# HiLab-git/FPL-plus

Hardware: AMD Instinct MI355X
Metric: 3D volumes/sec (train step, 80x160x160) (higher is better)
Workload: dtype bf16; 1 GPU; UNet3D-DSBN 32-base-ch bf16 (fp32 master weights), per-GPU batch 2x1x80x160x160 synthetic VS crops, DiceLoss + Adam, domain alternating per step; global_batch=2, parallelism=dp1, step=zero_grad+forward+loss+backward+allreduce+adam

## Files before the change

### fpl-plus_amd/csrc/common.h

```cpp
#pragma once
#include <hip/hip_runtime.h>
#include <math.h>
#include <stdint.h>
#include <stdio.h>
#include <stdarg.h>
#include <string.h>
#include "../../include/fplx.h"

typedef __bf16 bf16_t;

#define FPLX_WAVE 64

inline char* fplx_err_buf() {
  static thread_local char buf[512];
  return buf;
}
inline int fplx_fail(int code, const char* fmt, ...) {
  va_list ap;
  va_start(ap, fmt);
  vsnprintf(fplx_err_buf(), 512, fmt, ap);
  va_end(ap);
  return code;
}
inline int fplx_check_launch(const char* what) {
// ... 194 lines not shown
  FPLX_REQUIRE((need < 1 || s0) && (need < 2 || s1), FPLX_E_NULL, "%s: kind %d needs %d state buffer(s) here", who, kind, need);
  *ns = need;
  return FPLX_OK;
}
struct FplxBlock { int x, y, z; };
__device__ __forceinline__ FplxBlock fplx_xcd_block(int on) {
  FplxBlock b = {(int)blockIdx.x, (int)blockIdx.y, (int)blockIdx.z};
  if (!on) return b;
  const unsigned gx = gridDim.x, gy = gridDim.y, gz = gridDim.z, t = gx * gy * gz;
  const unsigned l = (blockIdx.z * gy + blockIdx.y) * gx + blockIdx.x;
  const unsigned xcd = l & 7u, q = t >> 3, r = t & 7u;
  const unsigned lp = xcd * q + (xcd < r ? xcd : r) + (l >> 3);
  const unsigned per = gy * gz, xq = lp / per, rem = lp - xq * per;
  b.x = __builtin_amdgcn_readfirstlane((int)xq);
  b.z = __builtin_amdgcn_readfirstlane((int)(rem / gy));
  b.y = __builtin_amdgcn_readfirstlane((int)(rem % gy));
  return b;
}
struct FplxTileRange { int64_t first, end, step; };
__device__ __forceinline__ FplxTileRange fplx_xcd_tiles(int64_t ntiles, int on) {
  FplxTileRange t = {(int64_t)blockIdx.x, ntiles, (int64_t)gridDim.x};
  if (!on || gridDim.x < 16) return t;
  const unsigned c = blockIdx.x & 7u, xcd = (blockIdx.y * gridDim.x + blockIdx.x) & 7u;
  const int64_t q = ntiles >> 3, r = ntiles & 7;
  const int64_t start = xcd * q + ((int64_t)xcd < r ? xcd : r);
  t.first = start + (blockIdx.x >> 3);
  t.end = start + q + ((int64_t)xcd < r ? 1 : 0);
  t.step = (gridDim.x - c + 7u) >> 3;
  return t;
}
template <typename... P, typename... A>
inline void fplx_launch(void (*kernel)(P...), dim3 grid, dim3 block, size_t lds, hipStream_t st, A... args) {
  if (lds) (void)hipFuncSetAttribute((const void*)kernel, hipFuncAttributeMaxDynamicSharedMemorySize, (int)lds);
  kernel<<<grid, block, lds, st>>>(args...);
}
#endif
#define FPLX_KNOB_LIST(X)                                                                                              \
  X(XCD, "xcd", 1)                                                    \
  X(BRICK, "brick", 1)                                    \
  X(BRICK_FILL, "brick_fill", 192)           \
  X(BRICK_GEO, "brick_geo", -1)                    \
  X(BRICK_KSPLIT, "brick_ksplit", 0)                                             \
  X(EDGE_BLOCKS, "edge_blocks", 1024)                             \
  X(STEM_ROWS, "stem_rows", 1)                                              \
  X(OUTCONV_T, "outconv_t", 1)                                 \
  X(OUTCONV_DGRAD_MFMA, "outconv_dgrad_mfma", 1)                                                                       \
  X(OUTCONV_FWD_ROWS, "outconv_fwd_rows", 1)  \
  X(OUTCONV_DGRAD_ROWS, "outconv_dgrad_rows", 1)  \
  X(PACK_TILED, "pack_tiled", 1)                                                                                       \
  X(PACK_MULTI, "pack_multi", 1)                                                                                       \
  X(MARCH, "march", 1)                           \
  X(MARCH64_FW, "march64_fw", 0)                                \
  X(MARCH_DS, "march_ds", 0)                                       \
  X(MARCH128, "march128", 1)                                                                                           \
  X(MARCH64_LW, "march64_lw", 1)            \
  X(MARCH32_V2, "march32_v2", 4)              \
  X(WG_COT_MINVOX, "wg_cot_minvox", 0)                                                                                 \
  X(WG_TW, "wg_tw", 0)                                                                                                 \
  X(WG_CIT, "wg_cit", 2)                                                                                               \
  X(WG_COT, "wg_cot", 2)                                                                                               \
  X(WG_DS, "wg_ds", 0)                                                                                                 \
  X(WG_VOX, "wg_vox", 1)                              \
  X(WG_ROLL, "wg_roll", 1)                     \
  X(WG_ROLL_GEO, "wg_roll_geo", 0)          \
  X(WG_ROLL_M16, "wg_roll_m16", 1)                 \
  X(WG_ROLL_MB, "wg_roll_mb", 1)            \
  X(WG_ROLL_CUS, "wg_roll_cus", 256)                                \
  X(WG_ROLL_OVH, "wg_roll_ovh", 9)                     \
  X(WG_ROLL_MINVOX, "wg_roll_minvox", 0)                                                   \
  X(WG_ROLL2D, "wg_roll2d", 1)              \
  X(WG_ROLL2D_OVH, "wg_roll2d_ovh", 3)      \
  X(WG_REDUCE_ROWS, "wg_reduce_rows", 8)    \
  X(WG_VOX_LW, "wg_vox_lw", 1)              \
  X(WG_VOX_CUS, "wg_vox_cus", 128)          \
  X(WG_VOX_MAXV, "wg_vox_maxv", 10000)         \
  X(TILE_NT, "tile_nt", 0)                                                                                             \
  X(TILE_KS, "tile_ks", 0)                                                                                             \
  X(MID_TILE, "mid_tile", 1)                                                                                           \
  X(DECONV_ROWS, "deconv_rows", 1)                                                                                     \
  X(DECONV_DGRAD_ROWS, "deconv_dgrad_rows", 1)   \
  X(ROWS_SMALL_DIV, "rows_small_div", 16)   \
  X(EW_GROUP, "ew_group", 1)                                                                                           \
  X(POOL_COL, "pool_col", 1)                         \
  X(EW_INFLIGHT, "ew_inflight", 2)          \
  X(EW_INFLIGHT_REDUCE, "ew_inflight_reduce", 2)
enum FplxKnobId {
#define FPLX_KNOB_ENUM(id, key, def) FPLX_K_##id,
  FPLX_KNOB_LIST(FPLX_KNOB_ENUM)
#undef FPLX_KNOB_ENUM
  FPLX_K_COUNT
};
extern "C" __attribute__((visibility("hidden"))) int64_t fplx_knob_values[FPLX_K_COUNT];
static inline int64_t fplx_knob(int id) { return __atomic_load_n(&fplx_knob_values[id], __ATOMIC_RELAXED); }
static inline int fplx_xcd_on() { return (int)fplx_knob(FPLX_K_XCD); }

static inline int fplx_rows_for(int64_t voxels) {
  constexpr int cap = 512;
  const int div = voxels <= 32768 ? (int)fplx_knob(FPLX_K_ROWS_SMALL_DIV) : 64;
  int64_t r = (voxels + div - 1) / div;
  if (r > cap) r = cap;
  if (r < 1) r = 1;
  return (int)r;
}
```

### fpl-plus_amd/csrc/elementwise.hip

```cpp
#include "common.h"
#include "philox.h"

namespace {

constexpr int EW_THREADS = 256;

template <typename T> struct Vec;
template <> struct Vec<float> {
  static constexpr int N = 4;
  typedef float4 raw;
  static __device__ __forceinline__ void load(const float* p, float (&v)[4]) {
    const float4 r = *reinterpret_cast<const float4*>(p);
    v[0] = r.x; v[1] = r.y; v[2] = r.z; v[3] = r.w;
  }
  static __device__ __forceinline__ void load_nt(const float* p, float (&v)[4]) { load(p, v); }
  static __device__ __forceinline__ void store(float* p, const float (&v)[4]) {
    *reinterpret_cast<float4*>(p) = make_float4(v[0], v[1], v[2], v[3]);
  }
};
template <> struct Vec<bf16_t> {
  static constexpr int N = 8;
  typedef __attribute__((ext_vector_type(8))) __bf16 raw;
  static __device__ __forceinline__ void load(const bf16_t* p, float (&v)[8]) {
    const raw r = *reinterpret_cast<const raw*>(p);
#pragma unroll
    for (int i = 0; i < 8; ++i) v[i] = (float)r[i];
  }
  static __device__ __forceinline__ void load_nt(const bf16_t* p, float (&v)[8]) {
    const raw r = __builtin_nontemporal_load(reinterpret_cast<const raw*>(p));
#pragma unroll
    for (int i = 0; i < 8; ++i) v[i] = (float)r[i];
  }
  static __device__ __forceinline__ void store(bf16_t* p, const float (&v)[8]) {
    raw r;
#pragma unroll
    for (int i = 0; i < 8; ++i) r[i] = (bf16_t)v[i];
    *reinterpret_cast<raw*>(p) = r;
  }
};

template <typename T, int VEC>
__device__ __forceinline__ void ldv(const T* p, float (&v)[VEC]) {
  if constexpr (VEC == 1) v[0] = Act<T>::ld(p);
  else Vec<T>::load(p, v);
}
template <typename T, int VEC>
__device__ __forceinline__ void ldv_nt(const T* p, float (&v)[VEC]) {
  if constexpr (VEC == 1) v[0] = Act<T>::ld(p);
  else Vec<T>::load_nt(p, v);
}
template <typename T, int VEC>
__device__ __forceinline__ void stv(T* p, const float (&v)[VEC]) {
  if constexpr (VEC == 1) Act<T>::st(p, v[0]);
  else Vec<T>::store(p, v);
}

template <int VEC>
__device__ __forceinline__ void keep_flags(int64_t e, uint32_t thr, uint32_t k0, uint32_t k1, uint32_t sid,
                                           bool (&keep)[VEC]) {
  if constexpr (VEC == 1) {
    const Philox4 r = philox4x32_10((uint32_t)(e >> 2), 0u, sid, 0u, k0, k1);
    keep[0] = r.v[e & 3] >= thr;
  } else {
#pragma unroll
    for (int g = 0; g < VEC / 4; ++g) {
      const Philox4 r = philox4x32_10((uint32_t)((e >> 2) + g), 0u, sid, 0u, k0, k1);
#pragma unroll
      for (int i = 0; i < 4; ++i) keep[g * 4 + i] = r.v[i] >= thr;
    }
  }
}

struct DropCfg { uint32_t thr, k0, k1, sid; float inv_keep; int on; };

inline DropCfg make_drop(float p, uint64_t seed, uint32_t sid) {
  DropCfg d;
  d.on = p > 0.f;
  d.thr = dropout_threshold(p);
  d.k0 = (uint32_t)seed;
  d.k1 = (uint32_t)(seed >> 32);
  d.sid = sid;
  d.inv_keep = d.on ? (float)(1.0 / (1.0 - (double)p)) : 1.f;
  return d;
}

constexpr int FIN_THREADS = 256;
__global__ void __launch_bounds__(FIN_THREADS)
bn_train_finalize_k(const float* __restrict__ stats, int rows, int C, double count,
                    const float* __restrict__ gamma, const float* __restrict__ beta,
                    float* __restrict__ rm, float* __restrict__ rv, int64_t* __restrict__ nbt,
                    float momentum, float eps, float* __restrict__ mean, float* __restrict__ rstd,
                    float* __restrict__ scale, float* __restrict__ shift) {
  const int c = blockIdx.x;
  double s1 = 0.0, s2 = 0.0;
  for (int r = threadIdx.x; r < rows; r += FIN_THREADS) {
    s1 += (double)stats[((int64_t)r * 2 + 0) * C + c];
    s2 += (double)stats[((int64_t)r * 2 + 1) * C + c];
  }
  s1 = wave_sum_d(s1);
  s2 = wave_sum_d(s2);
  __shared__ double wred[FIN_THREADS / 64][2];
  if ((threadIdx.x & 63) == 0) { wred[threadIdx.x >> 6][0] = s1; wred[threadIdx.x >> 6][1] = s2; }
  __syncthreads();
  if (threadIdx.x != 0) return;
  s1 = (wred[0][0] + wred[1][0]) + (wred[2][0] + wred[3][0]);
  s2 = (wred[0][1] + wred[1][1]) + (wred[2][1] + wred[3][1]);
  if (c == 0 && nbt) *nbt += 1;
  const double m = s1 / count;
  double var = s2 / count - m * m;
  if (var < 0.0) var = 0.0;
  const float rs = (float)(1.0 / sqrt(var + (double)eps));
  const float mf = (float)m;
  mean[c] = mf;
  rstd[c] = rs;
  const float sc = gamma[c] * rs;
  scale[c] = sc;
  shift[c] = beta[c] - mf * sc;
  if (rm) rm[c] = (1.f - momentum) * rm[c] + momentum * mf;
  if (rv) {
    const double unb = count > 1.0 ? var * count / (count - 1.0) : var;
    rv[c] = (1.f - momentum) * rv[c] + momentum * (float)unb;
  }
}

__global__ void bn_eval_prepare_k(const float* __restrict__ gamma, const float* __restrict__ beta,
                                  const float* __restrict__ rm, const float* __restrict__ rv, float eps, int C,
                                  float* __restrict__ scale, float* __restrict__ shift) {
  const int c = blockIdx.x * blockDim.x + threadIdx.x;
  if (c >= C) return;
  const float rs = 1.0f / sqrtf(rv[c] + eps);
  const float sc = gamma[c] * rs;
  scale[c] = sc;
  shift[c] = beta[c] - rm[c] * sc;
}

template <typename T, int VEC>
__global__ void __launch_bounds__(EW_THREADS)
bn_act_fwd_k(const T* __restrict__ y, int64_t ldy, T* __restrict__ out, int64_t ldo, const float* __restrict__ scale,
// ... 538 lines not shown
  __shared__ float red[EW_THREADS / 64 * 64][2 * VEC + 1];
  float* row = part + (int64_t)blockIdx.x * (2 * C + 1);
  for (int ofs = G; ofs < 64; ofs <<= 1) {
#pragma unroll
    for (int j = 0; j < VEC; ++j) { sdz[j] += __shfl_xor(sdz[j], ofs, 64); sdx[j] += __shfl_xor(sdx[j], ofs, 64); }
    sds += __shfl_xor(sds, ofs, 64);
  }
  const int lane = threadIdx.x & 63, wave = threadIdx.x >> 6;
  if (lane < G) {
#pragma unroll
    for (int j = 0; j < VEC; ++j) { red[wave * 64 + lane][j] = sdz[j]; red[wave * 64 + lane][VEC + j] = sdx[j]; }
    red[wave * 64 + lane][2 * VEC] = sds;
  }
  __syncthreads();
  if ((int)threadIdx.x < G) {
#pragma unroll
    for (int j = 0; j < VEC; ++j) {
      float t0 = 0.f, t1 = 0.f;
#pragma unroll
      for (int wv = 0; wv < EW_THREADS / 64; ++wv) { t0 += red[wv * 64 + threadIdx.x][j]; t1 += red[wv * 64 + threadIdx.x][VEC + j]; }
      row[c0 + j] = t0;
      row[C + c0 + j] = t1;
    }
  }
  if (threadIdx.x == 0) {
    float t = 0.f;
    for (int wv = 0; wv < EW_THREADS / 64; ++wv)
      for (int k = 0; k < G; ++k) t += red[wv * 64 + k][2 * VEC];
    row[2 * C] = t;
  }
}

template <typename T, int VEC>
__global__ void __launch_bounds__(EW_THREADS)
bn_act_pool_fwd_col_k(const T* __restrict__ y, int64_t ldy, T* __restrict__ out, int64_t ldo, T* __restrict__ pooled,
                      int64_t ldp, const float* __restrict__ scale, const float* __restrict__ shift,
                      const float* __restrict__ slope_p, int N, int D, int H, int W, int C, int pd) {
  const int G = C / VEC, VL = EW_THREADS / G;
  const int g = threadIdx.x % G, vl = threadIdx.x / G, c0 = g * VEC;
  const int Do = D / pd, Ho = H / 2;
  const unsigned units = (unsigned)N * Do * Ho * W;
  const float slope = *slope_p;
  float sc[VEC], sh[VEC];
#pragma unroll
  for (int j = 0; j < VEC; ++j) { sc[j] = scale[c0 + j]; sh[j] = shift[c0 + j]; }
  for (unsigned u = blockIdx.x * VL + vl; u < units; u += gridDim.x * VL) {
    unsigned q = u;
    const int w = (int)(q % (unsigned)W); q /= (unsigned)W;
    const int ho = (int)(q % (unsigned)Ho); q /= (unsigned)Ho;
    const int d_o = (int)(q % (unsigned)Do);
    const int64_t n = q / (unsigned)Do;
    float a[4][VEC], best[VEC];
    int64_t vis[4];
#pragma unroll
    for (int t = 0; t < 4; ++t) {
      if (t >= 2 * pd) break;
      vis[t] = ((n * D + pd * d_o + (t >> 1)) * H + 2 * ho + (t & 1)) * W + w;
      ldv_nt<T, VEC>(y + vis[t] * ldy + c0, a[t]);
    }
#pragma unroll
    for (int j = 0; j < VEC; ++j) best[j] = -INFINITY;
#pragma unroll
    for (int t = 0; t < 4; ++t) {
      if (t >= 2 * pd) break;
#pragma unroll
      for (int j = 0; j < VEC; ++j) {
        float z = fmaf(a[t][j], sc[j], sh[j]);
        z = z > 0.f ? z : z * slope;
        z = (float)(T)z;
        a[t][j] = z;
        best[j] = z > best[j] ? z : best[j];
      }
      stv<T, VEC>(out + vis[t] * ldo + c0, a[t]);
    }
#pragma unroll
    for (int j = 0; j < VEC; ++j) {
      const float o = __shfl_xor(best[j], G, 64);
      best[j] = o > best[j] ? o : best[j];
    }
    if (!(w & 1)) stv<T, VEC>(pooled + (int64_t)(u >> 1) * ldp + c0, best);
  }
}

template <typename T, int VEC>
__global__ void __launch_bounds__(EW_THREADS)
pool_bwd_bn_reduce_col_k(const T* __restrict__ y, int64_t ldy, const T* __restrict__ dy, int64_t lddy,
                         const T* __restrict__ dskip, int64_t lds, T* __restrict__ dx, int64_t ldo,
                         const float* __restrict__ mean, const float* __restrict__ rstd, const float* __restrict__ scale,
                         const float* __restrict__ shift, const float* __restrict__ slope_p, int N, int D, int H, int W, int C,
                         int pd, float* __restrict__ part) {
  const int G = C / VEC, VL = EW_THREADS / G;
  const int g = threadIdx.x % G, vl = threadIdx.x / G, c0 = g * VEC;
  const int Do = D / pd, Ho = H / 2;
  const unsigned units = (unsigned)N * Do * Ho * W;
  const float slope = *slope_p;
  float sdz[VEC], sdx[VEC], sds = 0.f, m[VEC], rs[VEC], sc[VEC], sh[VEC];
#pragma unroll
  for (int j = 0; j < VEC; ++j) {
    sdz[j] = sdx[j] = 0.f;
    m[j] = mean[c0 + j]; rs[j] = rstd[c0 + j]; sc[j] = scale[c0 + j]; sh[j] = shift[c0 + j];
  }
  for (unsigned u = blockIdx.x * VL + vl; u < units; u += gridDim.x * VL) {
    unsigned q = u;
    const int w = (int)(q % (unsigned)W); q /= (unsigned)W;
    const int ho = (int)(q % (unsigned)Ho); q /= (unsigned)Ho;
    const int d_o = (int)(q % (unsigned)Do);
    const int64_t n = q / (unsigned)Do;
    float gr[VEC], best[VEC], a[4][VEC], o[4][VEC];
    int arg[VEC];
    int64_t vis[4];
    ldv<T, VEC>(dy + (int64_t)(u >> 1) * lddy + c0, gr);
#pragma unroll
    for (int t = 0; t < 4; ++t) {
      if (t >= 2 * pd) break;
      vis[t] = ((n * D + pd * d_o + (t >> 1)) * H + 2 * ho + (t & 1)) * W + w;
      ldv<T, VEC>(y + vis[t] * ldy + c0, a[t]);
      if (dskip) ldv<T, VEC>(dskip + vis[t] * lds + c0, o[t]);
      else {
#pragma unroll
        for (int j = 0; j < VEC; ++j) o[t][j] = 0.f;
      }
    }
#pragma unroll
    for (int j = 0; j < VEC; ++j) { best[j] = -INFINITY; arg[j] = 8; }
#pragma unroll
    for (int t = 0; t < 4; ++t) {
      if (t >= 2 * pd) break;
#pragma unroll
      for (int j = 0; j < VEC; ++j) {
        float z = fmaf(a[t][j], sc[j], sh[j]);
        z = z > 0.f ? z : z * slope;
        z = (float)(T)z;
        if (z > best[j]) { best[j] = z; arg[j] = 2 * t + (w & 1); }
      }
    }
#pragma unroll
    for (int j = 0; j < VEC; ++j) {
      const float ob = __shfl_xor(best[j], G, 64);
      const int oa = __shfl_xor(arg[j], G, 64);
      if (ob > best[j] || (ob == best[j] && oa < arg[j])) arg[j] = -1;
    }
#pragma unroll
    for (int t = 0; t < 4; ++t) {
      if (t >= 2 * pd) break;
#pragma unroll
      for (int j = 0; j < VEC; ++j) {
        const float dv = (float)(T)(o[t][j] + ((arg[j] == 2 * t + (w & 1)) ? gr[j] : 0.f));
        o[t][j] = dv;
        const float z = fmaf(a[t][j], sc[j], sh[j]);
        const float dz = z > 0.f ? dv : dv * slope;
        sds += z > 0.f ? 0.f : dv * z;
        sdz[j] += dz;
        sdx[j] = fmaf(dz, (a[t][j] - m[j]) * rs[j], sdx[j]);
      }
      stv<T, VEC>(dx + vis[t] * ldo + c0, o[t]);
    }
  }
  __shared__ float red[EW_THREADS / 64 * 64][2 * VEC + 1];
  float* row = part + (int64_t)blockIdx.x * (2 * C + 1);
  for (int ofs = G; ofs < 64; ofs <<= 1) {
#pragma unroll
    for (int j = 0; j < VEC; ++j) { sdz[j] += __shfl_xor(sdz[j], ofs, 64); sdx[j] += __shfl_xor(sdx[j], ofs, 64); }
    sds += __shfl_xor(sds, ofs, 64);
  }
  const int lane = threadIdx.x & 63, wave = threadIdx.x >> 6;
  if (lane < G) {
#pragma unroll
    for (int j = 0; j < VEC; ++j) { red[wave * 64 + lane][j] = sdz[j]; red[wave * 64 + lane][VEC + j] = sdx[j]; }
    red[wave * 64 + lane][2 * VEC] = sds;
  }
  __syncthreads();
  if ((int)threadIdx.x < G) {
#pragma unroll
    for (int j = 0; j < VEC; ++j) {
      float t0 = 0.f, t1 = 0.f;
#pragma unroll
      for (int wv = 0; wv < EW_THREADS / 64; ++wv) { t0 += red[wv * 64 + threadIdx.x][j]; t1 += red[wv * 64 + threadIdx.x][VEC + j]; }
      row[c0 + j] = t0;
      row[C + c0 + j] = t1;
    }
  }
  if (threadIdx.x == 0) {
    float t = 0.f;
    for (int wv = 0; wv < EW_THREADS / 64; ++wv)
      for (int k = 0; k < G; ++k) t += red[wv * 64 + k][2 * VEC];
    row[2 * C] = t;
  }
}

template <int KIND, int NS, bool VEC>
__global__ void __launch_bounds__(EW_THREADS)
optim_k(float* __restrict__ p, const float* __restrict__ g, float* __restrict__ s0, float* __restrict__ s1, int64_t n,
        int64_t head, const FplxOptimConst c) {
  const int64_t tid = (int64_t)blockIdx.x * EW_THREADS + threadIdx.x, stride = (int64_t)gridDim.x * EW_THREADS;
  const int64_t nv = VEC ? (n - head) / 4 : 0, body_end = head + 4 * nv;
  for (int64_t i = tid; i < nv; i += stride) {
    const int64_t x = head + 4 * i;
    float4 pv = *reinterpret_cast<const float4*>(p + x);
    const float4 gv = *reinterpret_cast<const float4*>(g + x);
    float4 av = {0.f, 0.f, 0.f, 0.f}, bv = {0.f, 0.f, 0.f, 0.f};
    if (NS > 0) av = *reinterpret_cast<const float4*>(s0 + x);
    if (NS > 1) bv = *reinterpret_cast<const float4*>(s1 + x);
    fplx_optim_elem<KIND, NS>(pv.x, gv.x, av.x, bv.x, c);
    fplx_optim_elem<KIND, NS>(pv.y, gv.y, av.y, bv.y, c);
    fplx_optim_elem<KIND, NS>(pv.z, gv.z, av.z, bv.z, c);
    fplx_optim_elem<KIND, NS>(pv.w, gv.w, av.w, bv.w, c);
    if (NS > 0) *reinterpret_cast<float4*>(s0 + x) = av;
    if (NS > 1) *reinterpret_cast<float4*>(s1 + x) = bv;
    *reinterpret_cast<float4*>(p + x) = pv;
  }
  const int64_t rest = head + (n - body_end);
  for (int64_t j = tid; j < rest; j += stride) {
    const int64_t x = j < head ? j : body_end + (j - head);
    float pi = p[x], a = 0.f, b = 0.f;
    if (NS > 0) a = s0[x];
    if (NS > 1) b = s1[x];
    fplx_optim_elem<KIND, NS>(pi, g[x], a, b, c);
    if (NS > 0) s0[x] = a;
    if (NS > 1) s1[x] = b;
    p[x] = pi;
  }
}

template <typename T>
__global__ void __launch_bounds__(EW_THREADS)
channel_stats_k(const T* __restrict__ x, int64_t ld, int64_t V, int C, float* __restrict__ part) {
  const int c = blockIdx.y * 64 + (threadIdx.x & 63);
  const int vl = threadIdx.x >> 6;
  float s = 0.f, q = 0.f;
  if (c < C)
    for (int64_t v = (int64_t)blockIdx.x * 4 + vl; v < V; v += (int64_t)gridDim.x * 4) {
      const float a = Act<T>::ld(x + v * ld + c);
      s += a;
      q = fmaf(a, a, q);
    }
  __shared__ float red[4][2][64];
  red[vl][0][threadIdx.x & 63] = s;
  red[vl][1][threadIdx.x & 63] = q;
// ... 195 lines not shown
}

static int maxpool_bwd_impl(const void* x, int64_t ldx, const void* dy, int64_t ldy, const void* dskip, int64_t lds,
                            void* dx, int64_t ldo, int n, int d, int h, int w, int c, int dt, int pd, fplx_stream_t stream) {
  FPLX_REQUIRE(x && dy && dx, FPLX_E_NULL, "maxpool2_bwd: null pointer");
  FPLX_REQUIRE(n > 0 && c > 0 && d >= pd && h >= 2 && w >= 2 && !(d % pd) && !(h & 1) && !(w & 1), FPLX_E_BADSHAPE,
               "maxpool2_bwd: bad shape (even %sH,W required) %dx%dx%d", pd == 2 ? "D," : "", d, h, w);
  FPLX_REQUIRE(ldx >= c && ldy >= c && (!dskip || lds >= c) && ldo >= c, FPLX_E_BADSHAPE,
               "maxpool2_bwd: a leading dimension (%lld, %lld, %lld, %lld) is smaller than C = %d", (long long)ldx,
               (long long)ldy, (long long)lds, (long long)ldo, c);
  hipStream_t st = (hipStream_t)stream;
  const int64_t vo = (int64_t)n * (d / pd) * (h / 2) * (w / 2);
  if (dt == FPLX_F32) {
    const bool ok = vec_ok<float>(x, ldx, dy, ldy, dx, ldo, c) && vec_ok<float>(dskip, lds, nullptr, 0, nullptr, 0, c);
    DISPATCH_VEC(float, ok, maxpool2_bwd_k, <<<ew_grid(vo * (ok ? c / 4 : c)), EW_THREADS, 0, st>>>(
                                                (const float*)x, ldx, (const float*)dy, ldy, (const float*)dskip, lds,
                                                (float*)dx, ldo, n, d, h, w, c, pd));
  } else if (dt == FPLX_BF16) {
    const bool ok = vec_ok<bf16_t>(x, ldx, dy, ldy, dx, ldo, c) && vec_ok<bf16_t>(dskip, lds, nullptr, 0, nullptr, 0, c);
    DISPATCH_VEC(bf16_t, ok, maxpool2_bwd_k, <<<ew_grid(vo * (ok ? c / 8 : c)), EW_THREADS, 0, st>>>(
                                                 (const bf16_t*)x, ldx, (const bf16_t*)dy, ldy, (const bf16_t*)dskip,
                                                 lds, (bf16_t*)dx, ldo, n, d, h, w, c, pd));
  } else
    return fplx_fail(FPLX_E_BADDTYPE, "maxpool2_bwd: dtype %d", dt);
  return fplx_check_launch("maxpool2_bwd");
}

int fplx_maxpool2_fwd(const void* x, int64_t ldx, void* y, int64_t ldy, int n, int d, int h, int w, int c, int dt,
                      fplx_stream_t stream) {
  return maxpool_fwd_impl(x, ldx, y, ldy, n, d, h, w, c, dt, 2, stream);
}
int fplx_maxpool2_bwd(const void* x, int64_t ldx, const void* dy, int64_t ldy, const void* dskip, int64_t lds, void* dx,
                      int64_t ldo, int n, int d, int h, int w, int c, int dt, fplx_stream_t stream) {
  return maxpool_bwd_impl(x, ldx, dy, ldy, dskip, lds, dx, ldo, n, d, h, w, c, dt, 2, stream);
}
int fplx_maxpool122_fwd(const void* x, int64_t ldx, void* y, int64_t ldy, int n, int d, int h, int w, int c, int dt,
                        fplx_stream_t stream) {
  return maxpool_fwd_impl(x, ldx, y, ldy, n, d, h, w, c, dt, 1, stream);
}
int fplx_maxpool122_bwd(const void* x, int64_t ldx, const void* dy, int64_t ldy, const void* dskip, int64_t lds, void* dx,
                        int64_t ldo, int n, int d, int h, int w, int c, int dt, fplx_stream_t stream) {
  return maxpool_bwd_impl(x, ldx, dy, ldy, dskip, lds, dx, ldo, n, d, h, w, c, dt, 1, stream);
}

int fplx_bn_pool_fused_ok(int c, int dt) {
  const int g = c / 8;
  return dt == FPLX_BF16 && c % 8 == 0 && g >= 1 && g <= 64 && (g & (g - 1)) == 0 ? 1 : 0;
}

static int bn_pool_args_ok(const char* what, int n, int d, int h, int w, int c, int dt, int pd) {
  FPLX_REQUIRE(n > 0 && c > 0 && d >= pd && h >= 2 && w >= 2 && !(d % pd) && !(h & 1) && !(w & 1) && (pd == 1 || pd == 2),
               FPLX_E_BADSHAPE, "%s: bad shape", what);
  FPLX_REQUIRE(fplx_bn_pool_fused_ok(c, dt), FPLX_E_BADSHAPE, "%s: C=%d dtype %d not supported (fplx_bn_pool_fused_ok)", what, c, dt);
  return FPLX_OK;
}

int fplx_bn_act_pool_fwd(const void* y, int64_t ldy, void* out, int64_t ldo, void* pooled, int64_t ldp, const float* scale,
                         const float* shift, const float* slope, int n, int d, int h, int w, int c, int dt, int pd,
                         fplx_stream_t stream) {
  FPLX_REQUIRE(y && out && pooled && scale && shift && slope, FPLX_E_NULL, "bn_act_pool_fwd: null pointer");
  const int rc = bn_pool_args_ok("bn_act_pool_fwd", n, d, h, w, c, dt, pd);
  if (rc != FPLX_OK) return rc;
  FPLX_REQUIRE(vec_ok<bf16_t>(y, ldy, out, ldo, pooled, ldp, c), FPLX_E_BADSHAPE, "bn_act_pool_fwd: pointers / leading dimensions not 16-byte aligned");
  const int64_t vo = (int64_t)n * (d / pd) * (h / 2) * (w / 2);
  if (fplx_knob(FPLX_K_POOL_COL) && c / 8 <= 32 && 2 * vo < ((int64_t)1 << 31))
    bn_act_pool_fwd_col_k<bf16_t, 8><<<ew_grid(2 * vo * (c / 8)), EW_THREADS, 0, (hipStream_t)stream>>>(
        (const bf16_t*)y, ldy, (bf16_t*)out, ldo, (bf16_t*)pooled, ldp, scale, shift, slope, n, d, h, w, c, pd);
  else
  bn_act_pool_fwd_k<bf16_t, 8><<<ew_grid(vo * (c / 8)), EW_THREADS, 0, (hipStream_t)stream>>>(
      (const bf16_t*)y, ldy, (bf16_t*)out, ldo, (bf16_t*)pooled, ldp, scale, shift, slope, n, d, h, w, c, pd);
  return fplx_check_launch("bn_act_pool_fwd");
}

int fplx_pool_bwd_bn_reduce(const void* y, int64_t ldy, const void* dy, int64_t lddy, const void* dskip, int64_t lds, void* dx,
                            int64_t ldo, const float* mean, const float* rstd, const float* scale, const float* shift,
                            const float* slope, int n, int d, int h, int w, int c, int dt, int pd, float* part,
                            fplx_stream_t stream) {
  FPLX_REQUIRE(y && dy && dx && mean && rstd && scale && shift && slope && part, FPLX_E_NULL, "pool_bwd_bn_reduce: null pointer");
  const int rc = bn_pool_args_ok("pool_bwd_bn_reduce", n, d, h, w, c, dt, pd);
  if (rc != FPLX_OK) return rc;
  FPLX_REQUIRE(vec_ok<bf16_t>(y, ldy, dy, lddy, dx, ldo, c) && vec_ok<bf16_t>(dskip, lds, nullptr, 0, nullptr, 0, c), FPLX_E_BADSHAPE,
               "pool_bwd_bn_reduce: pointers / leading dimensions not 16-byte aligned");
  const int rows = fplx_rows_for((int64_t)n * d * h * w);
  if (fplx_knob(FPLX_K_POOL_COL) && c / 8 <= 32 && (int64_t)n * (d / pd) * (h / 2) * w < ((int64_t)1 << 31))
    pool_bwd_bn_reduce_col_k<bf16_t, 8><<<rows, EW_THREADS, 0, (hipStream_t)stream>>>(
        (const bf16_t*)y, ldy, (const bf16_t*)dy, lddy, (const bf16_t*)dskip, lds, (bf16_t*)dx, ldo, mean, rstd, scale, shift, slope, n,
        d, h, w, c, pd, part);
  else
  pool_bwd_bn_reduce_k<bf16_t, 8><<<rows, EW_THREADS, 0, (hipStream_t)stream>>>(
      (const bf16_t*)y, ldy, (const bf16_t*)dy, lddy, (const bf16_t*)dskip, lds, (bf16_t*)dx, ldo, mean, rstd, scale, shift, slope, n,
      d, h, w, c, pd, part);
  return fplx_check_launch("pool_bwd_bn_reduce");
}

static int optim_step_as(const char* who, int kind, float* p, const float* g, float* s0, float* s1, int64_t n, const float* hp,
                         int nhp, int step, float grad_scale, fplx_stream_t stream) {
  FPLX_REQUIRE(p && g, FPLX_E_NULL, "%s: null pointer", who);
  FPLX_REQUIRE(n > 0, FPLX_E_BADSHAPE, "%s: n=%lld", who, (long long)n);
  FplxOptimConst c;
  int ns = 0;
  const int rc = fplx_optim_consts(who, kind, hp, nhp, step, grad_scale, s0, s1, &c, &ns);
  if (rc != FPLX_OK) return rc;
  FPLX_REQUIRE((uintptr_t)p % 4 == 0 && (uintptr_t)g % 4 == 0 && (ns < 1 || (uintptr_t)s0 % 4 == 0) && (ns < 2 || (uintptr_t)s1 % 4 == 0),
               FPLX_E_BADSHAPE, "%s: the buffers must be 4-byte aligned", who);
  const uintptr_t ph = (uintptr_t)p % 16;
  int64_t head = (int64_t)((16 - ph) % 16) / 4;
  if (head > n) head = n;
  const bool vec = (uintptr_t)g % 16 == ph && (ns < 1 || (uintptr_t)s0 % 16 == ph) && (ns < 2 || (uintptr_t)s1 % 16 == ph);
  if (!vec) head = 0;
  const int grid = ew_grid(vec ? (n - head) / 4 + 6 : n);
  hipStream_t st = (hipStream_t)stream;
#define FPLX_OPTIM_LAUNCH(K, S)                                                                       \
  do {                                                                                                \
    if (vec) optim_k<K, S, true><<<grid, EW_THREADS, 0, st>>>(p, g, s0, s1, n, head, c);              \
    else optim_k<K, S, false><<<grid, EW_THREADS, 0, st>>>(p, g, s0, s1, n, head, c);                 \
  } while (0)
  FPLX_OPTIM_DISPATCH(kind, ns, FPLX_OPTIM_LAUNCH)
#undef FPLX_OPTIM_LAUNCH
  return fplx_check_launch(who);
}

int fplx_optim_step(int kind, float* p, const float* g, float* s0, float* s1, int64_t n, const float* hp, int nhp, int step,
                    float grad_scale, fplx_stream_t stream) {
  return optim_step_as("optim_step", kind, p, g, s0, s1, n, hp, nhp, step, grad_scale, stream);
}

int fplx_adam_step(float* p, const float* g, float* m, float* v, int64_t n, float lr, float beta1, float beta2,
                   float eps, float weight_decay, int step, float grad_scale, fplx_stream_t stream) {
  const float hp[5] = {lr, beta1, beta2, eps, weight_decay};
  return optim_step_as("adam_step", FPLX_OPT_ADAM, p, g, m, v, n, hp, 5, step, grad_scale, stream);
}

}
```

Baseline: 246.1 volumes/s.

## Software-pipeline pool backward BN-reduce column kernel with double-buffered loads

Adds a pipelined variant of the fused maxpool-backward/BN-reduce column kernel that prefetches the next unit's dy, y and skip vectors into raw registers while the current unit is consumed. It also replaces per-iteration div/mod index decoding with incremental carry-based advancement, and specializes on pool depth and skip presence as template parameters. Scheduling barriers and an opaque re-read keep the compiler from collapsing the two buffers. The goal is to hide global memory latency in this bandwidth-bound kernel, at the cost of higher register pressure, which may reduce occupancy.

```diff
diff --git a/fpl-plus_amd/csrc/common.h b/fpl-plus_amd/csrc/common.h
--- a/fpl-plus_amd/csrc/common.h
+++ b/fpl-plus_amd/csrc/common.h
@@ -300,6 +300,7 @@
   X(ROWS_SMALL_DIV, "rows_small_div", 16)   \
   X(EW_GROUP, "ew_group", 1)                                                                                           \
   X(POOL_COL, "pool_col", 1)                         \
+  X(POOL_BWD_PIPE, "pool_bwd_pipe", 1)      \
   X(EW_INFLIGHT, "ew_inflight", 2)          \
   X(EW_INFLIGHT_REDUCE, "ew_inflight_reduce", 2)
 enum FplxKnobId {
diff --git a/fpl-plus_amd/csrc/elementwise.hip b/fpl-plus_amd/csrc/elementwise.hip
--- a/fpl-plus_amd/csrc/elementwise.hip
+++ b/fpl-plus_amd/csrc/elementwise.hip
@@ -1,4 +1,5 @@
 #include "common.h"
+#include "gfx950.h"
 #include "philox.h"
 
 namespace {
@@ -14,6 +15,13 @@
     v[0] = r.x; v[1] = r.y; v[2] = r.z; v[3] = r.w;
   }
   static __device__ __forceinline__ void load_nt(const float* p, float (&v)[4]) { load(p, v); }
+  static __device__ __forceinline__ raw load_raw(const float* p) { return *reinterpret_cast<const float4*>(p); }
+  static __device__ __forceinline__ void unpack(const raw& r, float (&v)[4]) { v[0] = r.x; v[1] = r.y; v[2] = r.z; v[3] = r.w; }
+  static __device__ __forceinline__ raw again(const raw& r) {
+    u32x4 t = __builtin_bit_cast(u32x4, r);
+    opaque_v(t);
+    return __builtin_bit_cast(raw, t);
+  }
   static __device__ __forceinline__ void store(float* p, const float (&v)[4]) {
     *reinterpret_cast<float4*>(p) = make_float4(v[0], v[1], v[2], v[3]);
   }
@@ -31,6 +39,16 @@
 #pragma unroll
     for (int i = 0; i < 8; ++i) v[i] = (float)r[i];
   }
+  static __device__ __forceinline__ raw load_raw(const bf16_t* p) { return *reinterpret_cast<const raw*>(p); }
+  static __device__ __forceinline__ void unpack(const raw& r, float (&v)[8]) {
+#pragma unroll
+    for (int i = 0; i < 8; ++i) v[i] = (float)r[i];
+  }
+  static __device__ __forceinline__ raw again(const raw& r) {
+    u32x4 t = __builtin_bit_cast(u32x4, r);
+    opaque_v(t);
+    return __builtin_bit_cast(raw, t);
+  }
   static __device__ __forceinline__ void store(bf16_t* p, const float (&v)[8]) {
     raw r;
 #pragma unroll
@@ -54,6 +72,14 @@
   if constexpr (VEC == 1) Act<T>::st(p, v[0]);
   else Vec<T>::store(p, v);
 }
+
+template <typename T, int VEC>
+__device__ __forceinline__ void as_floats(const float (&x)[VEC], float (&v)[VEC]) {
+#pragma unroll
+  for (int j = 0; j < VEC; ++j) v[j] = x[j];
+}
+template <typename T, int VEC>
+__device__ __forceinline__ void as_floats(const typename Vec<T>::raw& x, float (&v)[VEC]) { Vec<T>::unpack(x, v); }
 
 template <int VEC>
 __device__ __forceinline__ void keep_flags(int64_t e, uint32_t thr, uint32_t k0, uint32_t k1, uint32_t sid,
@@ -758,7 +784,7 @@
   }
 }
 
-template <typename T, int VEC>
+template <typename T, int VEC, bool PIPE, int PD = 0, bool SKIP = false>
 __global__ void __launch_bounds__(EW_THREADS)
 pool_bwd_bn_reduce_col_k(const T* __restrict__ y, int64_t ldy, const T* __restrict__ dy, int64_t lddy,
                          const T* __restrict__ dskip, int64_t lds, T* __restrict__ dx, int64_t ldo,
@@ -769,6 +795,8 @@
   const int g = threadIdx.x % G, vl = threadIdx.x / G, c0 = g * VEC;
   const int Do = D / pd, Ho = H / 2;
   const unsigned units = (unsigned)N * Do * Ho * W;
+  const int64_t HW = (int64_t)H * W;
+  const int rows = PIPE ? 2 * PD : 2 * pd;
   const float slope = *slope_p;
   float sdz[VEC], sdx[VEC], sds = 0.f, m[VEC], rs[VEC], sc[VEC], sh[VEC];
 #pragma unroll
@@ -776,60 +804,141 @@
     sdz[j] = sdx[j] = 0.f;
     m[j] = mean[c0 + j]; rs[j] = rstd[c0 + j]; sc[j] = scale[c0 + j]; sh[j] = shift[c0 + j];
   }
-  for (unsigned u = blockIdx.x * VL + vl; u < units; u += gridDim.x * VL) {
-    unsigned q = u;
-    const int w = (int)(q % (unsigned)W); q /= (unsigned)W;
-    const int ho = (int)(q % (unsigned)Ho); q /= (unsigned)Ho;
-    const int d_o = (int)(q % (unsigned)Do);
-    const int64_t n = q / (unsigned)Do;
-    float gr[VEC], best[VEC], a[4][VEC], o[4][VEC];
+  auto consume = [&](int ww, int64_t base, const auto& gr_in, const auto& a_in, const auto& o_in) {
+    float best[VEC], gr[VEC];
     int arg[VEC];
-    int64_t vis[4];
-    ldv<T, VEC>(dy + (int64_t)(u >> 1) * lddy + c0, gr);
+#pragma unroll
+    for (int j = 0; j < VEC; ++j) { best[j] = -INFINITY; arg[j] = 8; }
 #pragma unroll
     for (int t = 0; t < 4; ++t) {
-      if (t >= 2 * pd) break;
-      vis[t] = ((n * D + pd * d_o + (t >> 1)) * H + 2 * ho + (t & 1)) * W + w;
-      ldv<T, VEC>(y + vis[t] * ldy + c0, a[t]);
-      if (dskip) ldv<T, VEC>(dskip + vis[t] * lds + c0, o[t]);
-      else {
-#pragma unroll
-        for (int j = 0; j < VEC; ++j) o[t][j] = 0.f;
-      }
-    }
-#pragma unroll
-    for (int j = 0; j < VEC; ++j) { best[j] = -INFINITY; arg[j] = 8; }
-#pragma unroll
-    for (int t = 0; t < 4; ++t) {
-      if (t >= 2 * pd) break;
+      if (t >= rows) break;
+      float a[VEC];
+      as_floats<T, VEC>(a_in[t], a);
 #pragma unroll
       for (int j = 0; j < VEC; ++j) {
-        float z = fmaf(a[t][j], sc[j], sh[j]);
+        float z = fmaf(a[j], sc[j], sh[j]);
         z = z > 0.f ? z : z * slope;
         z = (float)(T)z;
-        if (z > best[j]) { best[j] = z; arg[j] = 2 * t + (w & 1); }
+        if (z > best[j]) { best[j] = z; arg[j] = 2 * t + ww; }
       }
     }
 #pragma unroll
     for (int j = 0; j < VEC; ++j) {
       const float ob = __shfl_xor(best[j], G, 64);
       const int oa = __shfl_xor(arg[j], G, 64);
-      if (ob > best[j] || (ob == best[j] && oa < arg[j])) arg[j] = -1;
-    }
+      const bool other = PIPE ? (ob > best[j]) | ((ob == best[j]) & (oa < arg[j]))
+                              : ob > best[j] || (ob == best[j] && oa < arg[j]);
+      if (other) arg[j] = -1;
+    }
+    as_floats<T, VEC>(gr_in, gr);
 #pragma unroll
     for (int t = 0; t < 4; ++t) {
-      if (t >= 2 * pd) break;
+      if (t >= rows) break;
+      float a[VEC], o[VEC];
+      if constexpr (PIPE) {
+        __builtin_amdgcn_sched_barrier(0);
+        as_floats<T, VEC>(Vec<T>::again(a_in[t]), a);
+      } else
+        as_floats<T, VEC>(a_in[t], a);
+      as_floats<T, VEC>(o_in[t], o);
 #pragma unroll
       for (int j = 0; j < VEC; ++j) {
-        const float dv = (float)(T)(o[t][j] + ((arg[j] == 2 * t + (w & 1)) ? gr[j] : 0.f));
-        o[t][j] = dv;
-        const float z = fmaf(a[t][j], sc[j], sh[j]);
+        const float dv = (float)(T)(o[j] + ((arg[j] == 2 * t + ww) ? gr[j] : 0.f));
+        o[j] = dv;
+        const float z = fmaf(a[j], sc[j], sh[j]);
         const float dz = z > 0.f ? dv : dv * slope;
         sds += z > 0.f ? 0.f : dv * z;
         sdz[j] += dz;
-        sdx[j] = fmaf(dz, (a[t][j] - m[j]) * rs[j], sdx[j]);
+        sdx[j] = fmaf(dz, (a[j] - m[j]) * rs[j], sdx[j]);
       }
-      stv<T, VEC>(dx + vis[t] * ldo + c0, o[t]);
+      stv<T, VEC>(dx + (base + (t >> 1) * HW + (t & 1) * W) * ldo + c0, o);
+    }
+  };
+  const unsigned st = gridDim.x * VL;
+  unsigned u = blockIdx.x * VL + vl;
+  if constexpr (!PIPE) {
+    for (; u < units; u += st) {
+      unsigned q = u;
+      const int w = (int)(q % (unsigned)W); q /= (unsigned)W;
+      const int ho = (int)(q % (unsigned)Ho); q /= (unsigned)Ho;
+      const int d_o = (int)(q % (unsigned)Do);
+      const int64_t n = q / (unsigned)Do;
+      const int64_t base = ((n * D + pd * d_o) * H + 2 * ho) * W + w;
+      float gr[VEC], a[4][VEC], o[4][VEC];
+      ldv<T, VEC>(dy + (int64_t)(u >> 1) * lddy + c0, gr);
+#pragma unroll
+      for (int t = 0; t < 4; ++t) {
+        if (t >= 2 * pd) break;
+        const int64_t vi = base + (t >> 1) * HW + (t & 1) * W;
+        ldv<T, VEC>(y + vi * ldy + c0, a[t]);
+        if (dskip) ldv<T, VEC>(dskip + vi * lds + c0, o[t]);
+        else {
+#pragma unroll
+          for (int j = 0; j < VEC; ++j) o[t][j] = 0.f;
+        }
+      }
+      consume(w & 1, base, gr, a, o);
+    }
+  } else {
+    typedef typename Vec<T>::raw R;
+    struct Unit { R gr, a[4], o[4]; };
+    unsigned q = u;
+    int w = (int)(q % (unsigned)W); q /= (unsigned)W;
+    int ho = (int)(q % (unsigned)Ho); q /= (unsigned)Ho;
+    int d_o = (int)(q % (unsigned)Do);
+    int n = (int)(q / (unsigned)Do);
+    q = st;
+    const int sw = (int)(q % (unsigned)W); q /= (unsigned)W;
+    const int sho = (int)(q % (unsigned)Ho); q /= (unsigned)Ho;
+    const int sdo = (int)(q % (unsigned)Do);
+    const int sn = (int)(q / (unsigned)Do);
+    const int ww = w & 1;
+    auto fetch = [&](unsigned uu, int64_t base, Unit& x) {
+      x.gr = Vec<T>::load_raw(dy + (int64_t)(uu >> 1) * lddy + c0);
+#pragma unroll
+      for (int t = 0; t < 2 * PD; ++t) {
+        const int64_t vi = base + (t >> 1) * HW + (t & 1) * W;
+        x.a[t] = Vec<T>::load_raw(y + vi * ldy + c0);
+        if (SKIP) x.o[t] = Vec<T>::load_raw(dskip + vi * lds + c0);
+      }
+      __builtin_amdgcn_sched_barrier(0);
+    };
+    auto use = [&](int64_t base, const Unit& x) { consume(ww, base, x.gr, x.a, x.o); };
+    int64_t base = 0, bnext = 0;
+    auto base_of = [&]() { return ((int64_t)(n * D + PD * d_o) * H + 2 * ho) * W + w; };
+    auto advance = [&]() {
+      w += sw;
+      int cy = w >= W ? 1 : 0;
+      w -= cy ? W : 0;
+      ho += sho + cy;
+      cy = ho >= Ho ? 1 : 0;
+      ho -= cy ? Ho : 0;
+      d_o += sdo + cy;
+      cy = d_o >= Do ? 1 : 0;
+      d_o -= cy ? Do : 0;
+      n += sn + cy;
+      u += st;
+      base = bnext;
+      bnext = base_of();
+    };
+    if (u < units) {
+      Unit xa = {}, xb = {};
+      bnext = base_of();
+      fetch(u, bnext, xa);
+      advance();
+      bool last_b = false;
+      for (;;) {
+        if (u >= units) break;
+        fetch(u, bnext, xb);
+        use(base, xa);
+        advance();
+        if (u >= units) { last_b = true; break; }
+        fetch(u, bnext, xa);
+        use(base, xb);
+        advance();
+      }
+      if (last_b) use(base, xb);
+      else use(base, xa);
     }
   }
   __shared__ float red[EW_THREADS / 64 * 64][2 * VEC + 1];
@@ -1191,11 +1300,15 @@
   FPLX_REQUIRE(vec_ok<bf16_t>(y, ldy, dy, lddy, dx, ldo, c) && vec_ok<bf16_t>(dskip, lds, nullptr, 0, nullptr, 0, c), FPLX_E_BADSHAPE,
                "pool_bwd_bn_reduce: pointers / leading dimensions not 16-byte aligned");
   const int rows = fplx_rows_for((int64_t)n * d * h * w);
-  if (fplx_knob(FPLX_K_POOL_COL) && c / 8 <= 32 && (int64_t)n * (d / pd) * (h / 2) * w < ((int64_t)1 << 31))
-    pool_bwd_bn_reduce_col_k<bf16_t, 8><<<rows, EW_THREADS, 0, (hipStream_t)stream>>>(
+  if (fplx_knob(FPLX_K_POOL_COL) && c / 8 <= 32 && (int64_t)n * (d / pd) * (h / 2) * w < ((int64_t)1 << 31)) {
+    auto kern = pool_bwd_bn_reduce_col_k<bf16_t, 8, false>;
+    if (fplx_knob(FPLX_K_POOL_BWD_PIPE))
+      kern = pd == 2 ? (dskip ? pool_bwd_bn_reduce_col_k<bf16_t, 8, true, 2, true> : pool_bwd_bn_reduce_col_k<bf16_t, 8, true, 2, false>)
+                     : (dskip ? pool_bwd_bn_reduce_col_k<bf16_t, 8, true, 1, true> : pool_bwd_bn_reduce_col_k<bf16_t, 8, true, 1, false>);
+    kern<<<rows, EW_THREADS, 0, (hipStream_t)stream>>>(
         (const bf16_t*)y, ldy, (const bf16_t*)dy, lddy, (const bf16_t*)dskip, lds, (bf16_t*)dx, ldo, mean, rstd, scale, shift, slope, n,
         d, h, w, c, pd, part);
-  else
+  } else
   pool_bwd_bn_reduce_k<bf16_t, 8><<<rows, EW_THREADS, 0, (hipStream_t)stream>>>(
       (const bf16_t*)y, ldy, (const bf16_t*)dy, lddy, (const bf16_t*)dskip, lds, (bf16_t*)dx, ldo, mean, rstd, scale, shift, slope, n,
       d, h, w, c, pd, part);
```

Result: faster. 248.6 volumes/s, median of 6 (+1.0%).
